# doubleailes/crust-render

Measured on AMD Instinct MI355X. Metric: Mray/s (closest-hit + shadow queries) of the path-tracing integrator, higher is better.
Workload: dtype f32; 1 GPU; samples/cornellbox.usda 1920x1080, 512 spp per step per GPU-share (x1 GPUs), depth 32, triangle r=1, variance 0; 14 steps = 7168 spp; rays_total=33550217735, closest_hit=33550217735, camera_rays=14863564800, target_spp=1024

## Files before the change

### crust-render_amd/__init__.py

```python
import ctypes as C
import os
import subprocess

import numpy as np

_HERE = os.path.dirname(os.path.abspath(__file__))
LIB_PATH = os.environ.get("CRT_AMD_LIB") or os.path.join(_HERE, "libcrt_amd.so")
CSRC = os.path.join(_HERE, "csrc")

MASK_CAMERA, MASK_SHADOW, MASK_INDIRECT, MASK_ALL = 1, 2, 4, 0xFFFFFFFF
INVALID_ID = 0xFFFFFFFF
INF = float("inf")

CRT_OK = 0
_ERRORS = {-1: "CRT_ERR_BAD_ARG", -2: "CRT_ERR_BAD_ID", -3: "CRT_ERR_NO_DEVICE", -4: "CRT_ERR_STACK",
           -5: "CRT_ERR_UNSUPPORTED", -6: "CRT_ERR_NO_MEMORY"}


class CrtError(RuntimeError):
    def __init__(self, code, what=""):
        detail = ""
        try:
            detail = _lib.crt_last_error().decode() if _lib is not None else ""
        except Exception:
# ... 622 lines not shown
        _check(lib().crt_renderer_sample_counts(self.h, out.ctypes.data_as(C.POINTER(C.c_uint32))), "crt_renderer_sample_counts")
        return out

    def render_adaptive(self, spp, first=None, batch=4, stream=None):
        first = first or -(-max(self.settings.min_spp, 2) // 4) * 4
        s = 0
        while s < spp and self.active_pixels() > 0:
            n = min(first if s == 0 else batch, spp - s)
            self.render_samples(s, n, stream)
            s += n
        return s

    SHADE_CLASSES = ("emissive / escaped", "base", "coat / fuzz / thin film", "transmissive / subsurface")

    def shade_class_stats(self, enable=None):
        w, l = (C.c_uint64 * 4)(), (C.c_uint64 * 4)()
        _check(lib().crt_renderer_shade_class_stats(self.h, -1 if enable is None else int(bool(enable)), w, l),
               "crt_renderer_shade_class_stats")
        return {n: (int(w[k]), (l[k] / (64.0 * w[k])) if w[k] else 0.0) for k, n in enumerate(self.SHADE_CLASSES)}

    def pipeline(self):
        out = (C.c_uint32 * 3)()
        _check(lib().crt_renderer_pipeline(self.h, out), "crt_renderer_pipeline")
        return dict(fused=bool(out[0]), wide=bool(out[1]), grid=int(out[2]))

    def lanes(self):
        return int(lib().crt_renderer_lanes(self.h)) if hasattr(lib(), "crt_renderer_lanes") else 1

    def set_lanes(self, lanes):
        return _check(lib().crt_renderer_set_lanes(self.h, int(lanes)), "crt_renderer_set_lanes")

    def profile(self, enable=True):
        _check(lib().crt_renderer_profile(self.h, 1 if enable else 0), "crt_renderer_profile")

    def profile_read(self):
        ms = (C.c_double * 4)()
        n = (C.c_uint64 * 4)()
        _check(lib().crt_renderer_profile_read(self.h, ms, n), "crt_renderer_profile_read")
        names = ("extend", "shade", "shadow", "other")
        return {names[k]: dict(ms=float(ms[k]), launches=int(n[k])) for k in range(4)}


def scene_path(name):
    import os
    if str(name).startswith("synthetic:") or os.path.exists(name):
        return name
    base = os.path.join(os.path.dirname(os.path.dirname(os.path.abspath(__file__))), "scenes", name)
# ... 76 lines not shown
```

### crust-render_amd/csrc/crt_internal.h

```cpp
#pragma once

#include <atomic>
#include <cstddef>
#include <cstdint>
#include <memory>
#include <mutex>
#include <vector>

#include "../../include/crt.h"

namespace crt {

struct F3 {
  float x, y, z;
  float operator[](int i) const { return i == 0 ? x : (i == 1 ? y : z); }
  float &at(int i) { return i == 0 ? x : (i == 1 ? y : z); }
};
inline F3 f3(float x, float y, float z) { return F3{x, y, z}; }
inline F3 operator+(F3 a, F3 b) { return {a.x + b.x, a.y + b.y, a.z + b.z}; }
inline F3 operator-(F3 a, F3 b) { return {a.x - b.x, a.y - b.y, a.z - b.z}; }
inline F3 operator*(F3 a, float s) { return {a.x * s, a.y * s, a.z * s}; }
inline F3 operator-(F3 a) { return {-a.x, -a.y, -a.z}; }
inline float sse_min(float a, float b) { return a < b ? a : b; }
inline float sse_max(float a, float b) { return a > b ? a : b; }
// ... 175 lines not shown
  const int cold = (int)(s.cold & kColdAll);
  e.ext_cold = cold == 0 ? 0 : (cold == (int)kColdNormal ? (int)kColdNormal : (int)kColdAll);
  e.path_cold = cold == 0 ? 0 : (int)kColdAll;
  if (CRT_NOPK_BUILD && s.n_packets == 0 && e.direct) e.path_cold = (int)(kColdAll | kNoPackets);
  return CRT_OK;
}
inline bool engine_accepts(const EngineSelect &e, const DevScene &s, int kernel_cold) {
  if (s.direct_leaves != 0 && ((e.wide && !e.wide_direct) || !e.direct)) return false;
  if (e.wide_direct && s.direct_leaves == 0) return false;
  if ((kernel_cold & (int)kNoPackets) && (s.n_packets != 0 || s.direct_leaves == 0)) return false;
  return ((int)(s.cold & kColdAll) & ~kernel_cold) == 0;
}
int wide_request();

struct Knobs {
  int pool_stack_deep = -1;
  int direct_leaves = -1;
  int direct_inst = -1;
  int stage_roots = -1;
  uint32_t cold = 0;
  int inst_order = 1;
  int hot_packets = 1;
  int wide = -1;
  int mat_dedup = 1, partition = -1, simple = 1, prefer_stage = -1, cam_compact = 1, shade_wide = -1, fused = -1;
  int noclassify_from = 1 << 30, tail_from = 12, lanes = 4, grid_mult = 0;
  size_t max_batch_slots = 0, lane_min_paths = (size_t)96 << 20, stage_min_paths = (size_t)96 << 20;
};
Knobs read_knobs();
inline int select_engine_env(const DevScene &s, EngineSelect &e, bool renderer = false) {
  if (select_engine(s, wide_request(), e, renderer) == CRT_OK) return CRT_OK;
  return select_engine(s, -1, e, renderer);
}

struct DeviceImage {
  void *blob = nullptr;
  size_t bytes[7] = {0, 0, 0, 0, 0, 0, 0};
  uint32_t *err = nullptr;
  DevScene view{};
  ~DeviceImage();
};

struct Scene : std::enable_shared_from_this<Scene> {
  Bvh bvh;
  uint32_t n_geoms = 0;
  bool has_motion = false;
  uint32_t depth = 1;
  std::mutex dev_mu;
// ... 49 lines not shown
```

### crust-render_amd/csrc/kernels/pathtrace.hip

```cpp
#include <cstddef>
#include <cstdlib>
#include <cstring>
#include <new>
#include <string>
#include <unordered_map>
#include <vector>

#include "shade.hip.h"
#include "traverse_pool.hip.h"

namespace crt {

using namespace dev;

namespace {

#ifndef CRT_EXTEND_WAVES
#define CRT_EXTEND_WAVES 3
#endif
#ifndef CRT_SHADE_WAVES
#define CRT_SHADE_WAVES 3
#endif
#ifndef CRT_SHADOW_WAVES
#define CRT_SHADOW_WAVES 3
// ... 352 lines not shown
    return true;
  };
  auto emit = [&](uint32_t i, bool hit, const Hit &h, float dx, float dy, float dz) {
    if (hit) {
      const bool front = dot3(dx, dy, dz, h.nx, h.ny, h.nz) < 0.0f;
      st_hit(&H.h[i], make_float4(h.t, front ? h.nx : -h.nx, front ? h.ny : -h.ny, front ? h.nz : -h.nz));
      st_hit(&H.geom[i], h.geom | (front ? 0x80000000u : 0u));
    } else {
      st_hit(&H.geom[i], kInvalid);
    }
    done++;
  };
  run_traversal<false, STATS, WIDE, COLD, WIDE != 0>(P.scene, engine_lds, 0.001f, err, st, fetch, emit, mask);
  if (err) atomicOr(&C->err, err);
  if (STATS) flush_stats(st, tstats, done);
}
template <bool STATS, int WIDE, int COLD>
__global__ __launch_bounds__(kBlock, WIDE ? 4 : CRT_EXTEND_WAVES) void k_extend(Params P, PathSoA S, HitSoA H, Counters *C, int cur,
                                                                     int first, CrtTravStats *tstats) {
  __shared__ __attribute__((aligned(16))) uint32_t engine_lds[WIDE ? kEngineLdsWide : kEngineLdsDwords];
  extend_segment<STATS, WIDE, COLD, true>(P, S, H, C, cur, first, tstats, engine_lds);
}

template <int MATS, bool INF, bool LIT, int ARENA>
__device__ __forceinline__ void shade_segment(const Params &P, const PathSoA &S, const PathSoA &N, const HitSoA &H,
                                              const ShadowSoA &Q, Counters *C, int cur, float4 *staging,
                                              uint32_t *sobol_tab ,
                                              bool first ,
                                              bool all_pending = false ) {
  constexpr bool MEDIA = MATS == 2, SIMPLE = MATS == 0;
  constexpr bool COMPACT = CRT_CAM_COMPACT_BUILD && !LIT;
  constexpr bool MAT_INDEX = CRT_MAT_INDEX_BUILD && ARENA != kArenaWide;
  __shared__ uint32_t lds_ctr[10];
  __shared__ uint32_t out_n[kBins];
  __shared__ uint32_t pre[kBins + 1];
  bins_prefix(&C->seg[cur][blockIdx.x * kBins], pre);
  const uint32_t n = pre[kBins];
  if (n == 0) {
    if (threadIdx.x < kBins) C->seg[1 - cur][blockIdx.x * kBins + threadIdx.x] = 0;
    if (threadIdx.x == 0) C->shadow[blockIdx.x] = 0;
    return;
  }
  if (threadIdx.x < 10) lds_ctr[threadIdx.x] = 0;
  if (threadIdx.x < kBins) out_n[threadIdx.x] = 0;
  sobol_tables_init(sobol_tab);
  const CrtMaterial *mats = P.materials;
  if (P.n_materials <= (uint32_t)mat_lds_max(ARENA)) {
    uint32_t *dst = sobol_tab + kSobolLdsWords;
    const uint32_t *src = reinterpret_cast<const uint32_t *>(P.materials);
    const uint32_t words = P.n_materials * (uint32_t)(sizeof(CrtMaterial) / 4);
    for (uint32_t w = threadIdx.x; w < words; w += kBlock) dst[w] = src[w];
    mats = reinterpret_cast<const CrtMaterial *>(dst);
    __syncthreads();
  }
  const uint32_t seg0 = blockIdx.x * P.seg_cap;
  const uint32_t n_lights = LIT ? P.n_lights : 0u;
  uint32_t s_closest = 0, s_shadow = 0, s_vertices = 0, s_rr_t = 0, s_rr_k = 0, s_esc = 0, s_depth = 0;
  uint32_t *ring = sobol_tab + ARENA - kRingDwords;
  uint8_t *cls_lds = reinterpret_cast<uint8_t *>(ring) - kClassLdsMax;
  __shared__ uint32_t ring_tail[kClasses];
  const bool part = P.partition != 0;
  const bool cls_in_lds = part && P.n_materials <= (uint32_t)kClassLdsMax;
  if (threadIdx.x < kClasses) ring_tail[threadIdx.x] = 0;
  if (cls_in_lds)
    for (uint32_t g = threadIdx.x; g < P.n_materials; g += kBlock) cls_lds[g] = P.mat_class[g];
  __syncthreads();
  uint32_t next_in = 0;
  uint32_t head[kClasses], tail[kClasses];
#pragma unroll
  for (int c = 0; c < kClasses; c++) head[c] = 0;
  for (;;) {
#pragma unroll
    for (int c = 0; c < kClasses; c++) tail[c] = ring_tail[c];
    __syncthreads();
    auto most_pending = [&](int &c_best) {
      uint32_t best = tail[0] - head[0];
      c_best = 0;
#pragma unroll
      for (int c = 1; c < kClasses; c++)
        if (tail[c] - head[c] > best) { best = tail[c] - head[c]; c_best = c; }
      return best;
    };
    int c_sel;
    while (most_pending(c_sel) < (uint32_t)kBlock && next_in < n) {
      const uint32_t k_c = next_in + threadIdx.x;
      next_in += kBlock;
      bool pending = false;
      uint32_t cls = 0;
      if (all_pending && !part) pending = k_c < n;
      else if (k_c < n) {
        const uint32_t i_c = bin_slot(k_c, pre, P.seg_cap);
        const uint32_t hg = H.geom[i_c];
        uint4 D;
        float4 A, B, Cc = make_float4(1.0f, 0.0f, 0.0f, 0.0f);
        if (COMPACT && first && P.cam_compact) {
          float4 a = S.a[i_c];
          asm volatile("" : "+v"(a.x));
          compact_camera_path(P, k_c, a, A, B, D);
        } else if (!(kRegenFirst && first)) {
          D = S.d[i_c]; A = S.a[i_c]; B = S.b[i_c];
          if (!first) Cc = S.c[i_c];
          asm volatile("" : "+v"(A.x), "+v"(B.x), "+v"(Cc.x));
        } else {
          D = make_uint4(0u, 0u, (P.max_depth & 0xffffu) << 16, 0u);
          A = make_float4(0.0f, 0.0f, 0.0f, 0.0f); B = make_float4(0.0f, 0.0f, 1.0f, 1.0f);
          if (hg == kInvalid && P.max_depth > 0) {
            const CameraSample cs = camera_sample(P, camera_slot_sample(k_c), P.sample_begin, sobol_tab);
            A.w = cs.d.x; B.x = cs.d.y; B.y = cs.d.z;
            D.y = cs.pix; D.w = cs.sl;
          }
        }
        const int remaining = (int)(D.z >> 16);
        const bool carries_medium = MEDIA && (D.w >> kMediumShift) != 0;
        if (!INF && hg == kInvalid && remaining > 0 && !carries_medium) {
          const V3 rd = v3(A.w, B.x, B.y), beta = v3(B.z, B.w, Cc.x);
          V3 L = v3(Cc.y, Cc.z, Cc.w);
          s_closest++;
          s_esc++;
          const V3 unit_direction = normalize(rd);
          const V3 background = splat(0.0f) + sky_gradient(unit_direction);
          L = L + beta * background;
          st_nt(&staging[(D.w & 0xffffu) * P.n_act + D.y], make_float4(L.x, L.y, L.z, 0.0f));
        } else {
          pending = true;
          if (part && hg != kInvalid) {
            const uint32_t g = hg & 0x7fffffffu;
            const uint32_t mi_c = (MAT_INDEX && P.mat_index) ? (uint32_t)P.mat_index[g] : g;
            cls = cls_in_lds ? cls_lds[mi_c] : P.mat_class[mi_c];
          }
        }
      }
      if (part) {
#pragma unroll
        for (int c = 0; c < kClasses; c++) {
          const bool mine = pending && cls == (uint32_t)c;
          const uint32_t at = seg_append(mine, &ring_tail[c]);
          if (mine) ring[c * kRing + at % kRing] = k_c;
        }
      } else {
        const uint32_t at = seg_append(pending, &ring_tail[0]);
        if (pending) ring[at % kRing] = k_c;
      }
      __syncthreads();
#pragma unroll
      for (int c = 0; c < kClasses; c++) tail[c] = ring_tail[c];
      __syncthreads();
    }
    const uint32_t avail = most_pending(c_sel);
    if (avail == 0) break;
    const uint32_t take = avail < (uint32_t)kBlock ? avail : (uint32_t)kBlock;
    const bool active = threadIdx.x < take;
    uint32_t head_sel = head[0];
#pragma unroll
    for (int c = 1; c < kClasses; c++) head_sel = c_sel == c ? head[c] : head_sel;
    const uint32_t k_in = active ? ring[c_sel * kRing + (head_sel + threadIdx.x) % kRing] : 0;
#pragma unroll
    for (int c = 0; c < kClasses; c++) head[c] += c_sel == c ? take : 0u;
    const uint32_t i = active ? bin_slot(k_in, pre, P.seg_cap) : 0;
    bool alive = false, want_shadow = false;
    V3 L = splat(0.0f), beta = splat(1.0f);
    V3 n_o = splat(0.0f), n_d = splat(0.0f), sh_d = splat(0.0f), sh_c = splat(0.0f), hit_p = splat(0.0f);
    float n_ppdf = 0.0f, sh_tmax = 0.0f, time = 0.0f;
    uint32_t meta = 0, aux = 0, pix = 0, pattern = 0, n_med = 0;
    bool n_delta = false, n_prev_valid = true;
    if (active) {
      float4 A, B, Cc = make_float4(1.0f, 0.0f, 0.0f, 0.0f);
      uint4 D;
      if (COMPACT && first && P.cam_compact) {
        compact_camera_path(P, k_in, S.a[i], A, B, D);
// ... 25 lines not shown
      const uint32_t geom = hg & 0x7fffffffu;
      const uint32_t mat_i = (MAT_INDEX && has_hit && P.mat_index) ? (uint32_t)P.mat_index[geom] : geom;
      if (P.class_stats) {
        const uint32_t my = has_hit ? (uint32_t)P.mat_class[(MAT_INDEX && P.mat_index) ? (uint32_t)P.mat_index[geom] : geom] : 0u;
#pragma unroll
        for (int c = 0; c < kClasses; c++) {
          const unsigned long long m = __ballot(my == (uint32_t)c);
          if (m && (int)(threadIdx.x & 63) == __ffsll((long long)m) - 1) {
            atomicAdd(&C->cls_waves[c], 1ull);
            atomicAdd(&C->cls_lanes[c], (unsigned long long)__popcll(m));
          }
        }
      }
      HitRec rec;
      rec.front_face = ((hg >> 31) & 1u) != 0;
      rec.t = 0.0f; rec.normal = splat(0.0f); rec.p = splat(0.0f);
      if (has_hit) {
        const float4 hh = H.h[i];
        rec.t = hh.x;
        rec.normal = v3(hh.y, hh.z, hh.w);
        rec.p = ro + rd * rec.t;
      }
      hit_p = rec.p;

      auto emission_weight = [&]() -> float {
        if (prev_delta) return 1.0f;
        for (uint32_t k = 0; k < n_lights; k++) {
          if (P.lights[k].geom_id == geom) {
            const float4 E = S.e[i];
            const V3 from = v3(E.x, E.y, E.z);
            const float light_pdf = rmax(solid_angle_pdf(P.lights[k], from, rec.p) / (float)n_lights, 1e-6f);
            return bounce_weight(P.strategy, E.w, light_pdf);
          }
        }
        return 1.0f;
      };

      if (remaining <= 0) {
        s_depth++;
        if (prev_valid) {
          s_closest++;
          if (has_hit) {
            const CrtMaterial &mat = mats[mat_i];
            const float cos_o = fabs_(dot(normalize(rd), rec.normal));
            V3 emitted = mat_emitted_directional<SIMPLE>(mat, cos_o);
            if (len2(emitted) > 0.0f) {
// ... 93 lines not shown
            if (n_rec >= (uint32_t)kRrStartBounce) {
              s_rr_t++;
              const float p_survive = rclamp(max_elem(beta), kRrMinProb, 1.0f);
              if (p_survive < 1.0f) {
                if (draw_rnd1(new_domain(vdom, K_RR)) >= p_survive) {
                  survived = false;
                  s_rr_k++;
                } else {
                  beta = beta / p_survive;
                }
              }
            }
            if (survived) {
              alive = true;
              n_o = sample.origin; n_d = sample.dir; n_ppdf = sample.pdf; n_delta = sample.delta;
              n_med = (MEDIA && sample.medium) ? P.media[mat_i].id : 0u;
            }
          }
          s_vertices++;
        }
      }
    }

    uint32_t j = 0;
    {
      const uint32_t my_bin = dir_bin(n_d.x, n_d.y, n_d.z);
#pragma unroll
      for (int b = 0; b < kBins; b++) {
        const bool mine = alive && my_bin == (uint32_t)b;
        const uint32_t pos = seg_append(mine, &out_n[b]);
        if (mine) j = (blockIdx.x * kBins + b) * P.seg_cap + pos;
      }
    }
    const uint32_t sl = aux & 0xffffu;
    const uint32_t film_idx = sl * P.n_act + pix;
    if (alive) {
      st_nt(&N.a[j], make_float4(n_o.x, n_o.y, n_o.z, n_d.x));
      st_nt(&N.b[j], make_float4(n_d.y, n_d.z, beta.x, beta.y));
      st_nt(&N.c[j], make_float4(beta.z, L.x, L.y, L.z));
      st_nt(&N.d[j], make_uint4(pattern, pix, ((meta & 0xffffu) + 1u) | (((meta >> 16) - 1u) << 16),
                                sl | (n_prev_valid ? kPrevValid : 0u) | (n_delta ? kPrevDelta : 0u) | (n_med << kMediumShift)));
      if (n_lights) st_nt(&N.e[j], make_float4(hit_p.x, hit_p.y, hit_p.z, n_ppdf));
      if (P.has_motion) st_nt(&N.time[j], time);
    } else if (active) {
      st_nt(&staging[film_idx], make_float4(L.x, L.y, L.z, 0.0f));
    }
    const uint32_t q = seg0 + seg_append(want_shadow, &lds_ctr[1]);
    if (want_shadow) {
      st_nt(&Q.a[q], make_float4(hit_p.x, hit_p.y, hit_p.z, sh_tmax));
      st_nt(&Q.b[q], make_float4(sh_d.x, sh_d.y, sh_d.z, time));
      st_nt(&Q.c[q], make_float4(sh_c.x, sh_c.y, sh_c.z, __uint_as_float(alive ? j : (kFilmTarget | film_idx))));
    }
    __syncthreads();
  }
  add_stat(&lds_ctr[2], s_closest); add_stat(&lds_ctr[3], s_shadow); add_stat(&lds_ctr[4], s_vertices);
  add_stat(&lds_ctr[5], s_rr_t); add_stat(&lds_ctr[6], s_rr_k); add_stat(&lds_ctr[7], s_esc);
  add_stat(&lds_ctr[8], s_depth);
  __syncthreads();
  if (threadIdx.x == 0) {
    C->shadow[blockIdx.x] = lds_ctr[1];
  }
  if (threadIdx.x < kBins) {
    C->seg[1 - cur][blockIdx.x * kBins + threadIdx.x] = out_n[threadIdx.x];
    C->seg[cur][blockIdx.x * kBins + threadIdx.x] = 0;
  }
  if (threadIdx.x >= 1 && threadIdx.x <= 7 && lds_ctr[threadIdx.x + 1])
    atomicAdd(&C->stats[threadIdx.x], (unsigned long long)lds_ctr[threadIdx.x + 1]);
}
template <int MATS, bool INF, bool WIDE, bool LIT>
__global__ __launch_bounds__(kBlock, WIDE ? CRT_SHADE_WIDE_WAVES : CRT_SHADE_WAVES) void k_shade(Params P, PathSoA S, PathSoA N, HitSoA H, ShadowSoA Q,
                                                                   Counters *C, int cur, float4 *staging, int first) {
  static_assert(LIT || !INF, "lights at infinity are lights");
  constexpr int ARENA = WIDE ? kArenaWide : kArenaDwords;
  __shared__ uint32_t sobol_tab[ARENA];
  shade_segment<MATS, INF, LIT, ARENA>(P, S, N, H, Q, C, cur, staging, sobol_tab, (first & 1) != 0, (first & 2) != 0);
}

template <bool STATS, int WIDE>
__device__ __forceinline__ void shadow_segment(const Params &P, const PathSoA &N, const ShadowSoA &Q, Counters *C,
                                               float4 *staging, CrtTravStats *tstats, uint32_t *engine_lds) {
  const uint32_t n = ((const volatile uint32_t *)C->shadow)[blockIdx.x];
  if (n == 0) return;
  __shared__ uint32_t next;
  if (threadIdx.x == 0) next = 0;
  const uint32_t seg0 = blockIdx.x * P.seg_cap;
  LaneStats st = {};
  uint32_t err = 0, done = 0;
  auto fetch = [&](bool want, RayIn &in) -> bool {
    uint32_t k;
    if (!lds_take(want, &next, n, k)) return false;
    const uint32_t q = seg0 + k;
    const float4 A = Q.a[q], B = Q.b[q];
    in.ox = A.x; in.oy = A.y; in.oz = A.z; in.dx = B.x; in.dy = B.y; in.dz = B.z;
    in.time = B.w; in.mask = CRT_MASK_SHADOW; in.t_min = 0.001f; in.t_max = A.w; in.slot = q;
    return true;
  };
  auto emit = [&](uint32_t q, bool occ, const Hit &, float, float, float) {
    done++;
// ... 149 lines not shown
  int n_lanes = 4;
  int last_lanes = 1;
  size_t lane_min_paths = (size_t)96 << 20;
  hipEvent_t ev_start = nullptr;
  float4 *film = nullptr;
  CrtMaterial *d_materials = nullptr;
  uint8_t *d_mat_class = nullptr;
  uint16_t *d_mat_index = nullptr;
  DevMedium *d_media = nullptr;
  bool has_media = false;
  int mats_kind = 1;
  PixelStats *d_pstats = nullptr;
  uint32_t *d_state = nullptr, *d_active = nullptr, *d_count = nullptr;
  uint32_t n_act = 0, min_spp = 2;
  float variance_threshold = 0.0f;
  EngineSelect engine;
  bool wide = false;
  bool prefer_stage = false;
  bool cam_compact_ok = true;
  int shade_wide = -1;
  size_t max_batch_slots = 0;
  int tail_from = 12;
  int noclassify_from = 1 << 30;
  int force_fused = -1;
  size_t stage_min_paths = (size_t)96 << 20;
  bool fused = true;
  int cus = 256, fused_mult = 3, stage_mult = 8, mult_forced = 0;
  CrtLight *d_lights = nullptr;
  uint32_t *d_pixels = nullptr;
  int grid = 768;
  hipStream_t last_stream = nullptr;
  bool profile = false;
  struct Ev { hipEvent_t a, b; int cls; };
  std::vector<Ev> events;
  double prof_ms[4] = {0, 0, 0, 0};
  uint64_t prof_launches[4] = {0, 0, 0, 0};

  ~Renderer() {
    drain_events();
    for (Lane &B : lanes) {
      if (B.stream) (void)hipStreamSynchronize(B.stream);
      if (B.blob) (void)hipFree(B.blob);
      if (B.C) (void)hipFree(B.C);
      if (B.stream) (void)hipStreamDestroy(B.stream);
      if (B.done) (void)hipEventDestroy(B.done);
    }
// ... 137 lines not shown

  int plan_lane(Lane &B, Params &p, uint32_t n_samples, CrtTravStats *d_tstats) {
    const size_t total = (size_t)p.n_act * n_samples;
    fused = force_fused >= 0 ? force_fused != 0 : !(prefer_stage && total >= stage_min_paths);
    if (d_tstats) fused = false;
    if (P.has_inf_lights) fused = false;
    grid = batch_grid(total, fused);
    p.seg_cap = (uint32_t)(((total + (size_t)grid * kBlock - 1) / ((size_t)grid * kBlock)) * kBlock);
    return ensure_buffers(B, (size_t)p.seg_cap * grid);
  }

  int render_lane(Lane &B, uint32_t sample_begin, uint32_t n_samples, hipStream_t st, CrtTravStats *d_tstats, bool fold_here) {
    PathSoA (&S)[2] = B.S;
    HitSoA &H = B.H;
    ShadowSoA &Q = B.Q;
    Counters *C = B.C;
    const bool adaptive = variance_threshold > 0.0f;
    if (adaptive && n_act == 0) return CRT_OK;
    Params p = P;
    p.sample_begin = sample_begin;
    p.n_act = adaptive ? n_act : P.n_pix;
    p.active = (adaptive && n_act < P.n_pix) ? d_active : nullptr;
    if (const int rc = plan_lane(B, p, n_samples, d_tstats)) return rc;
    float4 *staging = B.staging;
    const bool wide = !fused && this->wide;
    const bool wdirect = wide && engine.wide_direct && CRT_WIDE_DIRECT_BUILD != 0;
    p.cam_compact = (CRT_CAM_COMPACT_BUILD && !fused && cam_compact_ok && P.n_lights == 0 && !(P.camera.lens_radius > 0.0f) && !P.has_motion) ? 1u : 0u;
    auto fold = [&]() -> int {
      if (!fold_here) return CRT_HIP_OK(hipGetLastError()) ? CRT_OK : CRT_ERR_NO_DEVICE;
      if (!adaptive) {
        timed(3, st, [&] { hipLaunchKernelGGL(k_resolve, dim3(grid), dim3(kBlock), 0, st, staging, P.n_pix, n_samples, film); });
        return CRT_HIP_OK(hipGetLastError()) ? CRT_OK : CRT_ERR_NO_DEVICE;
      }
      timed(3, st, [&] {
        hipLaunchKernelGGL(k_resolve_adaptive, dim3(grid), dim3(kBlock), 0, st, staging, p.active, p.n_act, n_samples, film,
                           d_pstats, d_state, min_spp, variance_threshold);
        (void)hipMemsetAsync(d_count, 0, 4, st);
        hipLaunchKernelGGL(k_compact_active, dim3(grid), dim3(kBlock), 0, st, d_state, P.n_pix, d_active, d_count);
      });
      uint32_t h = 0;
      if (!CRT_HIP_OK(hipMemcpyAsync(&h, d_count, 4, hipMemcpyDeviceToHost, st)) || !CRT_HIP_OK(hipStreamSynchronize(st)))
        return CRT_ERR_NO_DEVICE;
      n_act = h;
      return CRT_OK;
    };
    const bool lit = P.n_lights > 0;
// ... 54 lines not shown
            case 3: CRT_TAIL_NP(1, true); break;
            case 4: CRT_TAIL_NP(2, false); break;
            default: CRT_TAIL_NP(2, true); break;
          }
#undef CRT_TAIL_NP
#undef CRT_TAIL
        });
        break;
      }
#define CRT_EXTEND(ST, W, CO) \
  timed(0, st, [&] { hipLaunchKernelGGL((k_extend<ST, W, CO>), dim3(grid), dim3(kBlock), 0, st, p, S[cur], H, C, cur, it == 0 ? 1 : 0, d_tstats); })
      if (d_tstats) { if (wide && !wdirect) CRT_EXTEND(true, 1, kColdAll); else CRT_EXTEND(true, 0, kColdAll); }
#if CRT_WIDE_DIRECT_BUILD
      else if (wdirect) { if (ext_cold == 0) CRT_EXTEND(false, 2, 0); else if (ext_cold == (int)kColdNormal) CRT_EXTEND(false, 2, kColdNormal); else CRT_EXTEND(false, 2, kColdAll); }
#endif
      else if (wide) { if (ext_cold == 0) CRT_EXTEND(false, 1, 0); else if (ext_cold == (int)kColdNormal) CRT_EXTEND(false, 1, kColdNormal); else CRT_EXTEND(false, 1, kColdAll); }
      else { if (ext_cold == 0) CRT_EXTEND(false, 0, 0); else if (ext_cold == (int)kColdNormal) CRT_EXTEND(false, 0, kColdNormal); else CRT_EXTEND(false, 0, kColdAll); }
#undef CRT_EXTEND
#define CRT_SHADE(M, I, W, L) \
  timed(1, st, [&] { hipLaunchKernelGGL((k_shade<M, I, W, L>), dim3(grid), dim3(kBlock), 0, st, p, S[cur], S[1 - cur], H, Q, C, cur, staging, (it == 0 ? 1 : 0) | ((int)it >= noclassify_from ? 2 : 0)); })
      if (mats_kind == 2) { if (P.has_inf_lights) CRT_SHADE(2, true, false, true); else if (lit) CRT_SHADE(2, false, false, true); else CRT_SHADE(2, false, false, false); }
      else if (mats_kind == 1) { if (P.has_inf_lights) CRT_SHADE(1, true, false, true); else if (lit) CRT_SHADE(1, false, false, true); else CRT_SHADE(1, false, false, false); }
      else if (P.has_inf_lights) CRT_SHADE(0, true, false, true);
      else if (wide && !P.mat_index && shade_wide != 0) { if (lit) CRT_SHADE(0, false, true, true); else CRT_SHADE(0, false, true, false); }
      else { if (lit) CRT_SHADE(0, false, false, true); else CRT_SHADE(0, false, false, false); }
#undef CRT_SHADE
      if (P.n_lights > 0 && P.strategy != CRT_STRATEGY_BSDF) {
#define CRT_SHADOW(ST, W) \
  timed(2, st, [&] { hipLaunchKernelGGL((k_shadow<ST, W>), dim3(grid), dim3(kBlock), 0, st, p, S[1 - cur], Q, C, staging, d_tstats ? d_tstats + 1 : nullptr); })
        if (d_tstats) { if (wide && !wdirect) CRT_SHADOW(true, 1); else CRT_SHADOW(true, 0); }
#if CRT_WIDE_DIRECT_BUILD
        else if (wdirect) CRT_SHADOW(false, 2);
#endif
        else { if (wide) CRT_SHADOW(false, 1); else CRT_SHADOW(false, 0); }
#undef CRT_SHADOW
      }
      cur = 1 - cur;
    }
    return fold();
  }
};

}

struct CrtRenderer { crt::Renderer r; };

using namespace crt;
// ... 139 lines not shown
  }
  if (!ok) return nullptr;
  {
    bool simple = true;
    for (size_t k = 0; k < n_materials; k++) simple = simple && material_class(materials[k]) <= 1;
    simple = simple && knobs.simple != 0;
    r.mats_kind = r.has_media ? 2 : (simple ? 0 : 1);
  }
  P.materials = r.d_materials; P.lights = r.d_lights; P.pixel_index = r.d_pixels;
  P.mat_class = r.d_mat_class;
  P.media = r.d_media; P.media_by_id = r.d_media ? r.d_media + n_materials : nullptr;
  hipDeviceProp_t prop;
  int dev = 0;
  (void)hipGetDevice(&dev);
  if (select_engine_env(P.scene, r.engine, true) != CRT_OK) {
    set_error_text("crt_renderer_new: no traversal-engine instance of this build can decode the scene image");
    return nullptr;
  }
  r.wide = r.engine.wide;
  r.prefer_stage = true;
  if (knobs.prefer_stage >= 0) r.prefer_stage = knobs.prefer_stage != 0;
  r.cam_compact_ok = knobs.cam_compact != 0;
  r.noclassify_from = knobs.noclassify_from;
  r.tail_from = knobs.tail_from;
  r.max_batch_slots = knobs.max_batch_slots;
  r.n_lanes = knobs.lanes < 1 ? 1 : (knobs.lanes > Renderer::kMaxLanes ? Renderer::kMaxLanes : knobs.lanes);
  r.lane_min_paths = knobs.lane_min_paths;
  r.shade_wide = knobs.shade_wide;
  r.force_fused = knobs.fused;
  r.stage_min_paths = knobs.stage_min_paths;
  if (hipGetDeviceProperties(&prop, dev) == hipSuccess && prop.multiProcessorCount > 0) r.cus = prop.multiProcessorCount;
  r.stage_mult = r.wide ? 8 : 3;
  if (knobs.grid_mult > 0) { r.fused_mult = r.stage_mult = knobs.grid_mult; r.mult_forced = 1; }
  r.fused = r.force_fused >= 0 ? r.force_fused != 0 : !r.prefer_stage;
  r.grid = r.batch_grid(0, r.fused);
  hold.p = nullptr;
  return R;
}
CrtRenderer *crt_renderer_new(CrtScene *scene, const CrtMaterial *materials, size_t n_materials, const CrtLight *lights,
                              size_t n_lights, const CrtCamera *camera, const CrtRenderSettings *settings,
                              uint32_t tile_rank, uint32_t tile_world) {
  CrtRenderer *R = nullptr;
  (void)abi_guard("crt_renderer_new", [&] {
    R = renderer_new(scene, materials, n_materials, lights, n_lights, camera, settings, tile_rank, tile_world);
    return (int)CRT_OK;
  });
// ... 93 lines not shown
  Renderer &R = r->r;
  if (out_waves && out_lanes) {
    unsigned long long h[8];
    if (!CRT_HIP_OK(hipStreamSynchronize(R.last_stream))) return CRT_ERR_NO_DEVICE;
    for (int c = 0; c < 4; c++) out_waves[c] = out_lanes[c] = 0;
    for (Renderer::Lane &B : R.lanes) {
      if (!CRT_HIP_OK(hipMemcpy(h, B.C->cls_waves, sizeof h, hipMemcpyDeviceToHost))) return CRT_ERR_NO_DEVICE;
      if (!CRT_HIP_OK(hipMemset(B.C->cls_waves, 0, sizeof h))) return CRT_ERR_NO_DEVICE;
      for (int c = 0; c < 4; c++) { out_waves[c] += h[c]; out_lanes[c] += h[4 + c]; }
    }
  }
  if (enable >= 0) R.P.class_stats = enable ? 1u : 0u;
  return CRT_OK;
}
int crt_renderer_lanes(const CrtRenderer *r) { return r ? r->r.last_lanes : 0; }
int crt_renderer_set_lanes(CrtRenderer *r, int lanes) {
  if (!r) return CRT_ERR_BAD_ARG;
  r->r.n_lanes = lanes < 1 ? 1 : (lanes > Renderer::kMaxLanes ? Renderer::kMaxLanes : lanes);
  return r->r.n_lanes;
}
int crt_renderer_pipeline(const CrtRenderer *r, uint32_t out[3]) {
  if (!r || !out) return CRT_ERR_BAD_ARG;
  out[0] = r->r.fused ? 1u : 0u;
  out[1] = (!r->r.fused && r->r.wide) ? 1u : 0u;
  out[2] = (uint32_t)r->r.grid;
  return CRT_OK;
}
int crt_renderer_profile(CrtRenderer *r, int enable) {
  if (!r) return CRT_ERR_BAD_ARG;
  r->r.drain_events();
  r->r.profile = enable != 0;
  for (int k = 0; k < 4; k++) { r->r.prof_ms[k] = 0; r->r.prof_launches[k] = 0; }
  return CRT_OK;
}
int crt_renderer_profile_read(CrtRenderer *r, double out_ms[4], uint64_t out_launches[4]) {
  if (!r || !out_ms || !out_launches) return CRT_ERR_BAD_ARG;
  r->r.drain_events();
  for (int k = 0; k < 4; k++) { out_ms[k] = r->r.prof_ms[k]; out_launches[k] = r->r.prof_launches[k]; }
  return CRT_OK;
}

}
```

### crust-render_amd/csrc/scene.cpp

```cpp
#include <hip/hip_runtime.h>

#include <cstdarg>
#include <cstdio>
#include <cmath>
#include <cstring>
#include <algorithm>
#include <utility>
#include <unordered_map>

#include <cstdlib>
#include "crt_internal.h"

namespace crt {

static F3 mat3_mul(const Mat3 &m, F3 r) {
  F3 res = m.x * r.x;
  res = res + m.y * r.y;
  res = res + m.z * r.z;
  return res;
}
Mat3 mat3_transpose(const Mat3 &m) {
  return {f3(m.x.x, m.y.x, m.z.x), f3(m.x.y, m.y.y, m.z.y), f3(m.x.z, m.y.z, m.z.z)};
}
static Mat3 mat3_inverse(const Mat3 &m) {
// ... 135 lines not shown
    const char *e = getenv(name);
    if (!e || !*e) return false;
    char *end = nullptr;
    const long long v = strtoll(e, &end, 10);
    if (end == e) return false;
    out = v;
    return true;
  };
  long long v;
  if (num("CRT_POOL_STACK_RT", v)) k.pool_stack_deep = v >= CRT_POOL_STACK_DEEP ? 1 : 0;
  if (num("CRT_DIRECT_LEAVES", v)) k.direct_leaves = v != 0;
  if (num("CRT_DIRECT_INST", v)) k.direct_inst = v != 0;
  if (num("CRT_STAGE_ROOTS", v)) k.stage_roots = (int)std::min<long long>(std::max<long long>(v, 0), 1 << 20);
  if (num("CRT_COLD", v)) k.cold = (uint32_t)v & kColdAll;
  if (num("CRT_INST_ORDER", v)) k.inst_order = v != 0;
  if (num("CRT_HOT_PACKETS", v)) k.hot_packets = v != 0;
  if (num("CRT_WIDE", v)) k.wide = v == 2 ? 2 : (v != 0);
  if (num("CRT_MAT_DEDUP", v)) k.mat_dedup = v != 0;
  if (num("CRT_PARTITION", v)) k.partition = v != 0;
  if (num("CRT_SIMPLE", v)) k.simple = v != 0;
  if (num("CRT_PREFER_STAGE", v)) k.prefer_stage = v != 0;
  if (num("CRT_CAM_COMPACT", v)) k.cam_compact = v != 0;
  if (num("CRT_SHADE_WIDE", v)) k.shade_wide = v != 0;
  if (num("CRT_FUSED", v)) k.fused = v != 0;
  if (num("CRT_NOCLASSIFY_FROM", v)) k.noclassify_from = (int)std::min<long long>(std::max<long long>(v, 0), 1 << 30);
  if (num("CRT_TAIL_FROM", v)) k.tail_from = (int)std::min<long long>(std::max<long long>(v, 0), 1 << 30);
  if (num("CRT_LANES", v)) k.lanes = (int)std::min<long long>(std::max<long long>(v, 1), 4);
  if (num("CRT_GRID_MULT", v)) k.grid_mult = (int)std::min<long long>(std::max<long long>(v, 0), 64);
  if (num("CRT_MAX_BATCH_SLOTS", v)) k.max_batch_slots = v > 0 ? (size_t)v : 0;
  if (num("CRT_LANE_MIN_PATHS", v)) k.lane_min_paths = v > 0 ? (size_t)v : 1;
  if (num("CRT_STAGE_MIN_PATHS", v)) k.stage_min_paths = v > 0 ? (size_t)v : 1;
  return k;
}
int wide_request() { return read_knobs().wide; }

int device_ok() {
  static int ok = [] {
    int n = 0;
    if (!CRT_HIP_OK(hipGetDeviceCount(&n)) || n <= 0) return 0;
    return 1;
  }();
  return ok;
}

namespace {
struct Flat {
// ... 458 lines not shown
```

Measured before the change: 10630 Mray/s.

## Add software-pipelined shade kernel prefetching path state into LDS via async DMA

Adds a specialized shade kernel for simple, unlit, non-motion scenes. It splits paths into hit and miss rings and prefetches the next batch's path and hit records into per-wave LDS staging with global_load_lds, so those loads overlap shading of the current batch. Materials are copied into LDS, and the ring/classification logic is simplified to two classes. It also adds optional cycle-counter stamps for profiling. The cost is heavy LDS use and a narrow applicability gate, with fallback to the existing kernel otherwise.

```diff
diff --git a/crust-render_amd/__init__.py b/crust-render_amd/__init__.py
--- a/crust-render_amd/__init__.py
+++ b/crust-render_amd/__init__.py
@@ -668,7 +668,7 @@
     def pipeline(self):
         out = (C.c_uint32 * 3)()
         _check(lib().crt_renderer_pipeline(self.h, out), "crt_renderer_pipeline")
-        return dict(fused=bool(out[0]), wide=bool(out[1]), grid=int(out[2]))
+        return dict(fused=bool(out[0]), wide=bool(out[1] & 1), shade_pipe=bool(out[1] & 2), grid=int(out[2]))
 
     def lanes(self):
         return int(lib().crt_renderer_lanes(self.h)) if hasattr(lib(), "crt_renderer_lanes") else 1
diff --git a/crust-render_amd/csrc/crt_internal.h b/crust-render_amd/csrc/crt_internal.h
--- a/crust-render_amd/csrc/crt_internal.h
+++ b/crust-render_amd/csrc/crt_internal.h
@@ -221,7 +221,7 @@
   int inst_order = 1;
   int hot_packets = 1;
   int wide = -1;
-  int mat_dedup = 1, partition = -1, simple = 1, prefer_stage = -1, cam_compact = 1, shade_wide = -1, fused = -1;
+  int mat_dedup = 1, partition = -1, simple = 1, prefer_stage = -1, cam_compact = 1, shade_wide = -1, shade_pipe = 1, fused = -1;
   int noclassify_from = 1 << 30, tail_from = 12, lanes = 4, grid_mult = 0;
   size_t max_batch_slots = 0, lane_min_paths = (size_t)96 << 20, stage_min_paths = (size_t)96 << 20;
 };
diff --git a/crust-render_amd/csrc/kernels/pathtrace.hip b/crust-render_amd/csrc/kernels/pathtrace.hip
--- a/crust-render_amd/csrc/kernels/pathtrace.hip
+++ b/crust-render_amd/csrc/kernels/pathtrace.hip
@@ -398,6 +398,9 @@
   extend_segment<STATS, WIDE, COLD, true>(P, S, H, C, cur, first, tstats, engine_lds);
 }
 
+#ifndef CRT_SHADE_STAMPS
+#define CRT_SHADE_STAMPS 0
+#endif
 template <int MATS, bool INF, bool LIT, int ARENA>
 __device__ __forceinline__ void shade_segment(const Params &P, const PathSoA &S, const PathSoA &N, const HitSoA &H,
                                               const ShadowSoA &Q, Counters *C, int cur, float4 *staging,
@@ -443,12 +446,23 @@
   __syncthreads();
   uint32_t next_in = 0;
   uint32_t head[kClasses], tail[kClasses];
+  constexpr bool STAMPS = CRT_SHADE_STAMPS != 0 && ARENA == kArenaWide;
+  unsigned long long t_acc[8] = {0, 0, 0, 0, 0, 0, 0, 0}, t0 = STAMPS ? __builtin_readcyclecounter() : 0ull;
+  auto lap = [&](int slot, bool drain) {
+    if (STAMPS) {
+      if (drain) asm volatile("s_waitcnt vmcnt(0)" ::: "memory");
+      const unsigned long long t = __builtin_readcyclecounter();
+      t_acc[slot] += t - t0;
+      t0 = t;
+    }
+  };
 #pragma unroll
   for (int c = 0; c < kClasses; c++) head[c] = 0;
   for (;;) {
 #pragma unroll
     for (int c = 0; c < kClasses; c++) tail[c] = ring_tail[c];
     __syncthreads();
+    lap(2, false);
     auto most_pending = [&](int &c_best) {
       uint32_t best = tail[0] - head[0];
       c_best = 0;
@@ -472,11 +486,13 @@
         if (COMPACT && first && P.cam_compact) {
           float4 a = S.a[i_c];
           asm volatile("" : "+v"(a.x));
+          if (STAMPS) asm volatile("s_waitcnt vmcnt(0)" : "+v"(a.x) : : "memory");
           compact_camera_path(P, k_c, a, A, B, D);
         } else if (!(kRegenFirst && first)) {
           D = S.d[i_c]; A = S.a[i_c]; B = S.b[i_c];
           if (!first) Cc = S.c[i_c];
           asm volatile("" : "+v"(A.x), "+v"(B.x), "+v"(Cc.x));
+          if (STAMPS) asm volatile("s_waitcnt vmcnt(0)" : "+v"(A.x), "+v"(D.x) : : "memory");
         } else {
           D = make_uint4(0u, 0u, (P.max_depth & 0xffffu) << 16, 0u);
           A = make_float4(0.0f, 0.0f, 0.0f, 0.0f); B = make_float4(0.0f, 0.0f, 1.0f, 1.0f);
@@ -486,6 +502,7 @@
             D.y = cs.pix; D.w = cs.sl;
           }
         }
+        lap(0, false);
         const int remaining = (int)(D.z >> 16);
         const bool carries_medium = MEDIA && (D.w >> kMediumShift) != 0;
         if (!INF && hg == kInvalid && remaining > 0 && !carries_medium) {
@@ -517,10 +534,13 @@
         const uint32_t at = seg_append(pending, &ring_tail[0]);
         if (pending) ring[at % kRing] = k_c;
       }
+      lap(1, false);
       __syncthreads();
 #pragma unroll
       for (int c = 0; c < kClasses; c++) tail[c] = ring_tail[c];
       __syncthreads();
+      lap(2, false);
+      if (STAMPS) t_acc[7]++;
     }
     const uint32_t avail = most_pending(c_sel);
     if (avail == 0) break;
@@ -592,6 +612,8 @@
         rec.p = ro + rd * rec.t;
       }
       hit_p = rec.p;
+      if (STAMPS) asm volatile("" : "+v"(hit_p.x), "+v"(beta.x), "+v"(L.x), "+v"(pattern));
+      lap(3, true);
 
       auto emission_weight = [&]() -> float {
         if (prev_delta) return 1.0f;
@@ -731,6 +753,7 @@
       }
     }
 
+    lap(4, false);
     uint32_t j = 0;
     {
       const uint32_t my_bin = dir_bin(n_d.x, n_d.y, n_d.z);
@@ -760,8 +783,13 @@
       st_nt(&Q.b[q], make_float4(sh_d.x, sh_d.y, sh_d.z, time));
       st_nt(&Q.c[q], make_float4(sh_c.x, sh_c.y, sh_c.z, __uint_as_float(alive ? j : (kFilmTarget | film_idx))));
     }
+    lap(5, false);
     __syncthreads();
-  }
+    lap(2, false);
+    if (STAMPS) t_acc[6]++;
+  }
+  if (STAMPS && (threadIdx.x & 63) == 0)
+    for (int s = 0; s < 8; s++) atomicAdd(s < 4 ? &C->cls_waves[s] : &C->cls_lanes[s - 4], t_acc[s]);
   add_stat(&lds_ctr[2], s_closest); add_stat(&lds_ctr[3], s_shadow); add_stat(&lds_ctr[4], s_vertices);
   add_stat(&lds_ctr[5], s_rr_t); add_stat(&lds_ctr[6], s_rr_k); add_stat(&lds_ctr[7], s_esc);
   add_stat(&lds_ctr[8], s_depth);
@@ -783,6 +811,263 @@
   constexpr int ARENA = WIDE ? kArenaWide : kArenaDwords;
   __shared__ uint32_t sobol_tab[ARENA];
   shade_segment<MATS, INF, LIT, ARENA>(P, S, N, H, Q, C, cur, staging, sobol_tab, (first & 1) != 0, (first & 2) != 0);
+}
+
+constexpr uint32_t kPipeRing = 2 * kBlock;
+constexpr int kPipePlanes = 5;
+constexpr int kPipeWaveDwords = kPipePlanes * 256 + 64;
+constexpr int kPipeStageDwords = (kBlock / 64) * kPipeWaveDwords;
+constexpr int kPipeRingDwords = 2 * (int)kPipeRing;
+constexpr int kMatDwords = (int)(sizeof(CrtMaterial) / 4);
+constexpr int kPipeMatMax = (kArenaWide - kSobolLdsWords - kPipeRingDwords - kPipeStageDwords) / kMatDwords;
+static_assert(kPipeMatMax >= 6 && kSobolLdsWords + kPipeMatMax * kMatDwords + kPipeRingDwords + kPipeStageDwords <= kArenaWide,
+              "Sobol tables + material table + rings + staging blocks fit the four-wave arena");
+static_assert((kArenaWide - kPipeStageDwords) % 4 == 0 && kPipeWaveDwords % 4 == 0, "staging planes are 16-byte aligned");
+constexpr bool kShadePipeBuild = kBins == 1 && !kRegenFirst && CRT_SHADE_WIDE_WAVES == 4;
+#ifndef CRT_SHADE_PIPE_HIT_REGS
+#define CRT_SHADE_PIPE_HIT_REGS 0
+#endif
+
+typedef __attribute__((address_space(3))) void lds_void;
+__device__ __forceinline__ void lds_dma16(const void *src, uint32_t *lds_dst ) {
+  __builtin_amdgcn_global_load_lds(src, (lds_void *)lds_dst, 16, 0, 0);
+}
+__device__ __forceinline__ void lds_dma4(const void *src, uint32_t *lds_dst ) {
+  __builtin_amdgcn_global_load_lds(src, (lds_void *)lds_dst, 4, 0, 0);
+}
+__device__ __forceinline__ void lds_barrier() {
+  asm volatile("s_waitcnt lgkmcnt(0)" ::: "memory");
+  __builtin_amdgcn_s_barrier();
+  asm volatile("" ::: "memory");
+}
+__device__ __forceinline__ uint32_t uniform(uint32_t v) { return (uint32_t)__builtin_amdgcn_readfirstlane((int)v); }
+
+__device__ __forceinline__ void shade_segment_pipe(const Params &P, const PathSoA &S, const PathSoA &N, const HitSoA &H,
+                                                   Counters *C, int cur, float4 *staging, uint32_t *arena ,
+                                                   bool first) {
+  constexpr bool STAMPS = CRT_SHADE_STAMPS != 0;
+  __shared__ uint32_t lds_ctr[10];
+  __shared__ uint32_t out_n;
+  __shared__ uint32_t ring_tail[2];
+  const uint32_t n = uniform(((const volatile uint32_t *)C->seg[cur])[blockIdx.x]);
+  if (n == 0) {
+    if (threadIdx.x == 0) { C->seg[1 - cur][blockIdx.x] = 0; C->shadow[blockIdx.x] = 0; }
+    return;
+  }
+  if (threadIdx.x < 10) lds_ctr[threadIdx.x] = 0;
+  if (threadIdx.x == 0) out_n = 0;
+  if (threadIdx.x < 2) ring_tail[threadIdx.x] = 0;
+  sobol_tables_init(arena);
+  uint32_t *mat_lds = arena + kSobolLdsWords;
+  {
+    const uint32_t *src = reinterpret_cast<const uint32_t *>(P.materials);
+    const uint32_t words = P.n_materials * (uint32_t)kMatDwords;
+    for (uint32_t w = threadIdx.x; w < words; w += kBlock) mat_lds[w] = src[w];
+  }
+  const CrtMaterial *mats = reinterpret_cast<const CrtMaterial *>(mat_lds);
+  uint32_t *ring_h = arena + kArenaWide - kPipeStageDwords - kPipeRingDwords, *ring_m = ring_h + kPipeRing;
+  uint32_t *stg = arena + kArenaWide - kPipeStageDwords + (threadIdx.x >> 6) * kPipeWaveDwords;
+  const uint32_t lane = threadIdx.x & 63;
+  __syncthreads();
+  const uint32_t seg0 = blockIdx.x * P.seg_cap;
+  const bool compact = CRT_CAM_COMPACT_BUILD && first && P.cam_compact;
+  uint32_t s_closest = 0, s_vertices = 0, s_rr_t = 0, s_rr_k = 0, s_esc = 0, s_depth = 0;
+  unsigned long long t_acc[7] = {0, 0, 0, 0, 0, 0, 0}, t0 = 0;
+  auto lap = [&](int slot) {
+    if (STAMPS) { const unsigned long long t = __builtin_readcyclecounter(); t_acc[slot] += t - t0; t0 = t; }
+  };
+  uint32_t next_in = 0, head_h = 0, head_m = 0, tail_h = 0, tail_m = 0;
+  uint32_t hg_next = threadIdx.x < n ? H.geom[seg0 + threadIdx.x] : kInvalid;
+  uint32_t kind = 0, take = 0, k_in = 0;
+  if (STAMPS) t0 = __builtin_readcyclecounter();
+  for (;;) {
+    float4 A = make_float4(0.0f, 0.0f, 0.0f, 0.0f), B = make_float4(0.0f, 0.0f, 1.0f, 1.0f), Cc = make_float4(1.0f, 0.0f, 0.0f, 0.0f);
+    float4 hh = make_float4(0.0f, 0.0f, 0.0f, 0.0f);
+    uint4 D = make_uint4(0u, 0u, 0u, 0u);
+    uint32_t hg = kInvalid;
+    if (kind) {
+      asm volatile("s_waitcnt vmcnt(0)" ::: "memory");
+      A = reinterpret_cast<const float4 *>(stg)[lane];
+      if (!compact) {
+        B = reinterpret_cast<const float4 *>(stg + 256)[lane];
+        D = reinterpret_cast<const uint4 *>(stg + 768)[lane];
+        if (!first) Cc = reinterpret_cast<const float4 *>(stg + 512)[lane];
+      }
+      if (kind == 1 && CRT_SHADE_PIPE_HIT_REGS) {
+        hh = H.h[seg0 + k_in];
+        hg = H.geom[seg0 + k_in];
+      } else if (kind == 1) {
+        hh = reinterpret_cast<const float4 *>(stg + 1024)[lane];
+        hg = stg[1280 + lane];
+      }
+      asm volatile("s_waitcnt lgkmcnt(0)" ::: "memory");
+    }
+    lap(0);
+    while (next_in < n && tail_h - head_h < (uint32_t)kBlock && tail_m - head_m < (uint32_t)kBlock) {
+      lds_barrier();
+      const uint32_t k_c = next_in + threadIdx.x;
+      const uint32_t hg_c = hg_next;
+      next_in += kBlock;
+      hg_next = kInvalid;
+      if (next_in + threadIdx.x < n) hg_next = H.geom[seg0 + next_in + threadIdx.x];
+      const bool hit = k_c < n && hg_c != kInvalid, miss = k_c < n && hg_c == kInvalid;
+      const uint32_t at_h = seg_append(hit, &ring_tail[0]);
+      if (hit) ring_h[at_h % kPipeRing] = k_c;
+      const uint32_t at_m = seg_append(miss, &ring_tail[1]);
+      if (miss) ring_m[at_m % kPipeRing] = k_c;
+      lds_barrier();
+      tail_h = uniform(ring_tail[0]);
+      tail_m = uniform(ring_tail[1]);
+      if (STAMPS) t_acc[6]++;
+    }
+    lap(1);
+    const uint32_t pend_h = tail_h - head_h, pend_m = tail_m - head_m;
+    uint32_t kind_n = 0, take_n = 0, k_n = 0;
+    if (pend_h >= (uint32_t)kBlock || (pend_h && pend_m < (uint32_t)kBlock)) { kind_n = 1; take_n = pend_h < (uint32_t)kBlock ? pend_h : (uint32_t)kBlock; }
+    else if (pend_m) { kind_n = 2; take_n = pend_m < (uint32_t)kBlock ? pend_m : (uint32_t)kBlock; }
+    if (kind_n && threadIdx.x < take_n) {
+      k_n = kind_n == 1 ? ring_h[(head_h + threadIdx.x) % kPipeRing] : ring_m[(head_m + threadIdx.x) % kPipeRing];
+      const uint32_t i_n = seg0 + k_n;
+      lds_dma16(&S.a[i_n], stg);
+      if (!compact) {
+        lds_dma16(&S.b[i_n], stg + 256);
+        lds_dma16(&S.d[i_n], stg + 768);
+        if (!first) lds_dma16(&S.c[i_n], stg + 512);
+      }
+      if (kind_n == 1 && !CRT_SHADE_PIPE_HIT_REGS) {
+        lds_dma16(&H.h[i_n], stg + 1024);
+        lds_dma4(&H.geom[i_n], stg + 1280);
+      }
+    }
+    head_h += kind_n == 1 ? take_n : 0u;
+    head_m += kind_n == 2 ? take_n : 0u;
+    lap(2);
+    const bool active = threadIdx.x < take;
+    if (kind == 2) {
+      if (active) {
+        if (compact) compact_camera_path(P, k_in, A, A, B, D);
+        const int remaining = (int)(D.z >> 16);
+        const V3 rd = v3(A.w, B.x, B.y), beta = v3(B.z, B.w, Cc.x);
+        V3 L = v3(Cc.y, Cc.z, Cc.w);
+        if (remaining > 0) {
+          s_closest++;
+          s_esc++;
+          const V3 unit_direction = normalize(rd);
+          const V3 background = splat(0.0f) + sky_gradient(unit_direction);
+          L = L + beta * background;
+        } else {
+          s_depth++;
+          if ((D.w & kPrevValid) != 0) s_closest++;
+        }
+        st_nt(&staging[(D.w & 0xffffu) * P.n_act + D.y], make_float4(L.x, L.y, L.z, 0.0f));
+      }
+      lap(4);
+    } else if (kind == 1) {
+      bool alive = false;
+      V3 L = splat(0.0f), beta = splat(1.0f), n_o = splat(0.0f), n_d = splat(0.0f);
+      uint32_t meta = 0, aux = 0, pix = 0, pattern = 0;
+      bool n_delta = false;
+      if (active) {
+        if (compact) compact_camera_path(P, k_in, A, A, B, D);
+        const V3 ro = v3(A.x, A.y, A.z), rd = v3(A.w, B.x, B.y);
+        beta = v3(B.z, B.w, Cc.x);
+        L = v3(Cc.y, Cc.z, Cc.w);
+        pattern = D.x; pix = D.y; meta = D.z; aux = D.w;
+        const uint32_t n_rec = meta & 0xffffu;
+        const int remaining = (int)(meta >> 16);
+        const bool prev_valid = (aux & kPrevValid) != 0;
+        const uint32_t mat_i = hg & 0x7fffffffu;
+        HitRec rec;
+        rec.front_face = ((hg >> 31) & 1u) != 0;
+        rec.t = hh.x;
+        rec.normal = v3(hh.y, hh.z, hh.w);
+        rec.p = ro + rd * rec.t;
+        const CrtMaterial &mat = mats[mat_i];
+        const float emission_weight = 1.0f;
+        if (remaining <= 0) {
+          s_depth++;
+          if (prev_valid) {
+            s_closest++;
+            const float cos_o = fabs_(dot(normalize(rd), rec.normal));
+            const V3 emitted = mat_emitted_directional<true>(mat, cos_o);
+            if (len2(emitted) > 0.0f) L = L + beta * (emitted * emission_weight);
+          }
+        } else {
+          s_closest++;
+          const Sampler vdom = new_domain(Sampler{pattern, P.sample_begin + (aux & 0xffffu)}, (int)n_rec);
+          const V3 atten = splat(1.0f);
+          const float cos_o = fabs_(dot(normalize(rd), rec.normal));
+          const V3 emitted = mat_emitted_directional<true>(mat, cos_o);
+          V3 emit_here = splat(0.0f);
+          if (prev_valid) {
+            if (len2(emitted) > 0.0f) L = L + beta * ((atten * emitted) * emission_weight);
+          } else {
+            emit_here = emitted;
+          }
+          const V3 ba = beta * atten;
+          L = L + ba * emit_here;
+          Scatter sample;
+          if (mat_scatter<true>(mat, rd, rec, new_domain(vdom, K_BSDF), sample, arena)) {
+            const V3 dir = normalize(sample.dir);
+            const float cosine = sample.delta ? 1.0f : fabs_(dot(rec.normal, dir));
+            const V3 factor = (sample.value * cosine) / sample.pdf;
+            beta = beta * (atten * factor);
+            bool survived = true;
+            if (n_rec >= (uint32_t)kRrStartBounce) {
+              s_rr_t++;
+              const float p_survive = rclamp(max_elem(beta), kRrMinProb, 1.0f);
+              if (p_survive < 1.0f) {
+                if (draw_rnd1(new_domain(vdom, K_RR)) >= p_survive) {
+                  survived = false;
+                  s_rr_k++;
+                } else {
+                  beta = beta / p_survive;
+                }
+              }
+            }
+            if (survived) {
+              alive = true;
+              n_o = sample.origin; n_d = sample.dir; n_delta = sample.delta;
+            }
+          }
+          s_vertices++;
+        }
+      }
+      const uint32_t j = seg0 + seg_append(alive, &out_n);
+      const uint32_t sl = aux & 0xffffu;
+      if (alive) {
+        st_nt(&N.a[j], make_float4(n_o.x, n_o.y, n_o.z, n_d.x));
+        st_nt(&N.b[j], make_float4(n_d.y, n_d.z, beta.x, beta.y));
+        st_nt(&N.c[j], make_float4(beta.z, L.x, L.y, L.z));
+        st_nt(&N.d[j], make_uint4(pattern, pix, ((meta & 0xffffu) + 1u) | (((meta >> 16) - 1u) << 16),
+                                  sl | kPrevValid | (n_delta ? kPrevDelta : 0u)));
+      } else if (active) {
+        st_nt(&staging[sl * P.n_act + pix], make_float4(L.x, L.y, L.z, 0.0f));
+      }
+      lap(3);
+    }
+    if (STAMPS) t_acc[5]++;
+    if (!kind_n) break;
+    kind = kind_n; take = take_n; k_in = k_n;
+  }
+  add_stat(&lds_ctr[2], s_closest); add_stat(&lds_ctr[4], s_vertices);
+  add_stat(&lds_ctr[5], s_rr_t); add_stat(&lds_ctr[6], s_rr_k); add_stat(&lds_ctr[7], s_esc);
+  add_stat(&lds_ctr[8], s_depth);
+  __syncthreads();
+  if (threadIdx.x == 0) {
+    C->shadow[blockIdx.x] = 0;
+    C->seg[1 - cur][blockIdx.x] = out_n;
+    C->seg[cur][blockIdx.x] = 0;
+  }
+  if (threadIdx.x >= 1 && threadIdx.x <= 7 && lds_ctr[threadIdx.x + 1])
+    atomicAdd(&C->stats[threadIdx.x], (unsigned long long)lds_ctr[threadIdx.x + 1]);
+  if (STAMPS && lane == 0)
+    for (int s = 0; s < 7; s++) atomicAdd(s < 4 ? &C->cls_waves[s] : &C->cls_lanes[s - 4], t_acc[s]);
+}
+__global__ __launch_bounds__(kBlock, CRT_SHADE_WIDE_WAVES) void k_shade_pipe(Params P, PathSoA S, PathSoA N, HitSoA H, Counters *C,
+                                                                              int cur, float4 *staging, int first) {
+  __shared__ __attribute__((aligned(16))) uint32_t arena[kArenaWide];
+  shade_segment_pipe(P, S, N, H, C, cur, staging, arena, first != 0);
 }
 
 template <bool STATS, int WIDE>
@@ -978,6 +1263,12 @@
   size_t max_batch_slots = 0;
   int tail_from = 12;
   int noclassify_from = 1 << 30;
+  int shade_pipe = 1;
+  bool shade_piped = false;
+  bool shade_pipe_fits() const {
+    return kShadePipeBuild && shade_pipe != 0 && mats_kind == 0 && P.n_lights == 0 && !P.has_motion && !P.mat_index &&
+           P.partition == 0 && !P.class_stats && P.n_materials <= (uint32_t)kPipeMatMax;
+  }
   int force_fused = -1;
   size_t stage_min_paths = (size_t)96 << 20;
   bool fused = true;
@@ -1161,6 +1452,7 @@
     p.n_act = adaptive ? n_act : P.n_pix;
     p.active = (adaptive && n_act < P.n_pix) ? d_active : nullptr;
     if (const int rc = plan_lane(B, p, n_samples, d_tstats)) return rc;
+    shade_piped = false;
     float4 *staging = B.staging;
     const bool wide = !fused && this->wide;
     const bool wdirect = wide && engine.wide_direct && CRT_WIDE_DIRECT_BUILD != 0;
@@ -1261,7 +1553,14 @@
       if (mats_kind == 2) { if (P.has_inf_lights) CRT_SHADE(2, true, false, true); else if (lit) CRT_SHADE(2, false, false, true); else CRT_SHADE(2, false, false, false); }
       else if (mats_kind == 1) { if (P.has_inf_lights) CRT_SHADE(1, true, false, true); else if (lit) CRT_SHADE(1, false, false, true); else CRT_SHADE(1, false, false, false); }
       else if (P.has_inf_lights) CRT_SHADE(0, true, false, true);
-      else if (wide && !P.mat_index && shade_wide != 0) { if (lit) CRT_SHADE(0, false, true, true); else CRT_SHADE(0, false, true, false); }
+      else if (wide && !P.mat_index && shade_wide != 0) {
+        if (lit) CRT_SHADE(0, false, true, true);
+        else if (shade_pipe_fits() && (int)it < noclassify_from) {
+          shade_piped = true;
+          timed(1, st, [&] { hipLaunchKernelGGL(k_shade_pipe, dim3(grid), dim3(kBlock), 0, st, p, S[cur], S[1 - cur], H, C, cur, staging, it == 0 ? 1 : 0); });
+        }
+        else CRT_SHADE(0, false, true, false);
+      }
       else { if (lit) CRT_SHADE(0, false, false, true); else CRT_SHADE(0, false, false, false); }
 #undef CRT_SHADE
       if (P.n_lights > 0 && P.strategy != CRT_STRATEGY_BSDF) {
@@ -1447,6 +1746,7 @@
   if (knobs.prefer_stage >= 0) r.prefer_stage = knobs.prefer_stage != 0;
   r.cam_compact_ok = knobs.cam_compact != 0;
   r.noclassify_from = knobs.noclassify_from;
+  r.shade_pipe = knobs.shade_pipe;
   r.tail_from = knobs.tail_from;
   r.max_batch_slots = knobs.max_batch_slots;
   r.n_lanes = knobs.lanes < 1 ? 1 : (knobs.lanes > Renderer::kMaxLanes ? Renderer::kMaxLanes : knobs.lanes);
@@ -1586,7 +1886,7 @@
 int crt_renderer_pipeline(const CrtRenderer *r, uint32_t out[3]) {
   if (!r || !out) return CRT_ERR_BAD_ARG;
   out[0] = r->r.fused ? 1u : 0u;
-  out[1] = (!r->r.fused && r->r.wide) ? 1u : 0u;
+  out[1] = ((!r->r.fused && r->r.wide) ? 1u : 0u) | ((!r->r.fused && r->r.shade_piped) ? 2u : 0u);
   out[2] = (uint32_t)r->r.grid;
   return CRT_OK;
 }
diff --git a/crust-render_amd/csrc/scene.cpp b/crust-render_amd/csrc/scene.cpp
--- a/crust-render_amd/csrc/scene.cpp
+++ b/crust-render_amd/csrc/scene.cpp
@@ -181,6 +181,7 @@
   if (num("CRT_PREFER_STAGE", v)) k.prefer_stage = v != 0;
   if (num("CRT_CAM_COMPACT", v)) k.cam_compact = v != 0;
   if (num("CRT_SHADE_WIDE", v)) k.shade_wide = v != 0;
+  if (num("CRT_SHADE_PIPE", v)) k.shade_pipe = v != 0;
   if (num("CRT_FUSED", v)) k.fused = v != 0;
   if (num("CRT_NOCLASSIFY_FROM", v)) k.noclassify_from = (int)std::min<long long>(std::max<long long>(v, 0), 1 << 30);
   if (num("CRT_TAIL_FROM", v)) k.tail_from = (int)std::min<long long>(std::max<long long>(v, 0), 1 << 30);
```

Measured after the change: 10970 Mray/s, median of 6. 1.03x the previous value.
